# guangkun0818/speech2text

Measured on AMD Instinct MI355X. Metric: audio-seconds/sec (train step, zipformer pruned-RNN-T), higher is better.
Workload: dtype f32; 1 GPU; C3 zipformer pruned-RNN-T train step: chunk_size -1, 500 BPE, prune_range 5 (fbank+fwd+bwd+allreduce+ScaledAdam); accumulate_grad_batches=1, gemm_arith=bf16x2/3, per_gpu_batch=64, global_batch=64, labels_per_utt=50, parallelism=dp1

## Files before the change

include/s2t_mi355.h:

```cpp
#ifndef S2T_MI355_H_
#define S2T_MI355_H_

#ifdef __cplusplus
extern "C" {
#endif

int s2t_fbank_f32(const float* pcm, long pcm_stride, const long* num_samples, int batch,
                  const float* window400, const float* twiddle512, const int* mel_off,
                  const int* mel_k0, const float* mel_w, int nnz, int num_mel, float eps,
                  float scale_in, const float* cmvn_mean, const float* cmvn_istd, float* out,
                  int max_frames, long* out_frames, void* stream);

#define S2T_CTC_MAX_LABELS 1023
long s2t_ctc_workspace_floats(int B, int T, int Umax);
int s2t_ctc_loss_fwd_bwd(const float* logits, const long* targets, long tgt_stride,
                         const long* in_len, const long* tgt_len, int B, int T, int V, int Umax,
                         int blank, int zero_infinity, const float* grad_scale, float* workspace,
                         float* loss_per_utt, float* grad_logits, void* stream);

int s2t_fill_f32(float* p, long n, float v, void* stream);
int s2t_rnnt_row_exp(const float* x, long rows, int C, float* probs, float* rowmax, void* stream);
int s2t_rnnt_simple_pxpy(const float* am, const float* lm, const float* am_max,
                         const float* lm_max, const float* nrm, const long* symbols,
                         const long* boundary, int B, int S, int T, int C, int blank, float* px,
// ... 14 lines not shown
                         const float* lm_max, const float* nrm, const float* lm_sum,
                         const float* am_dot, const float* log_u, const long* symbols,
                         const long* boundary, int B, int S, int T, int C, int blank, float lam,
                         float mu, float* px, float* py, void* stream);
int s2t_rnnt_smooth_bwd(const float* am_probs, const float* lm_probs, const float* G_am,
                        const float* G_lm, const float* dpx, const float* dpy,
                        const float* gscale, const long* symbols, const float* lm_sum,
                        const float* am_dot, const float* u, int B, int S, int T, int C, int blank,
                        float lam, float mu, float* dlogu_part, float* v, float* d_am, float* d_lm,
                        void* stream);
int s2t_mutual_info_fwd(const float* px, const float* py, const long* boundary, int B, int S,
                        int T, float* p, float* ans, void* stream);
int s2t_mutual_info_bwd(const float* px, const float* py, const long* boundary, const float* p,
                        const float* ans_grad, int B, int S, int T, float* px_grad,
                        float* py_grad, void* stream);
int s2t_rnnt_prune_ranges(const float* px_grad, const float* py_grad, const long* boundary, int B,
                          int S, int T, int s_range, long* ranges, void* stream);
int s2t_rnnt_pruned_fwd(const float* am, const float* lm, const long* ranges,
                        const long* symbols, const long* boundary, int B, int S, int T, int C,
                        int R, int blank, int act, float* px, float* py, float* lse, void* stream);
int s2t_rnnt_pruned_bwd(const float* am, const float* lm, const long* ranges,
                        const long* symbols, const float* lse, const float* dpx, const float* dpy,
                        const float* gscale, int B, int S, int T, int C, int R, int blank, int act,
                        float* d_am, float* d_lm, int accumulate, void* stream);
int s2t_rnnt_lattice_fwd(const float* logits, const long* ranges, const long* symbols,
                         const long* boundary, int B, int S, int T, int V, int R, int blank,
                         float* px, float* py, float* lse, void* stream);
int s2t_rnnt_lattice_bwd(const float* logits, const long* ranges, const long* symbols,
                         const float* lse, const float* dpx, const float* dpy,
                         const float* gscale, int B, int S, int T, int V, int R, int blank,
                         float* d_logits, void* stream);


int s2t_swoosh_fwd(const float* x, float* y, long n, float offset, float constant, void* stream);
int s2t_swoosh_bwd(const float* x, const float* g, float* d, long n, float offset, void* stream);
int s2t_biasnorm_fwd(const float* x, const float* bias, const float* log_scale, long rows, int D,
                     float* y, float* scales, void* stream);
int s2t_biasnorm_fwd_tb(const float* x, const float* bias, const float* log_scale, int T, int B, int D,
                        float* y, float* scales, void* stream);
int s2t_biasnorm_bwd_tb(const float* x, const float* bias, const float* scales, const float* g, int T,
                        int B, int D, float* dx, float* dbias, float* dls, void* stream);
int s2t_norm_bypass_fwd(const float* x, const float* bias, const float* log_scale, const float* orig,
                        const float* bypass_scale, const float* fm, int B, long rows, int D, float* out,
                        float* scales, void* stream);
int s2t_norm_bypass_bwd(const float* x, const float* bias, const float* scales, const float* orig,
                        const float* bypass_scale, const float* g, const float* fm, int B, long rows, int D,
                        float* dx, float* d_orig, float* d_bypass_scale, float* dbias, float* dls,
                        void* stream);
int s2t_biasnorm_bwd(const float* x, const float* bias, const float* scales, const float* g,
                     long rows, int D, float* dx, float* dbias, float* dls, void* stream);
long s2t_balancer_bwd_workspace_floats(void);
int s2t_balancer_bwd(const float* x, long ldx, const float* g, long ldg, long rows, int C,
                     float min_mean, float max_mean, float min_rms, float max_rms,
                     float grad_scale, float* out, long ldo, float* workspace, int parity,
                     float act_off, void* stream);
int s2t_balancer_stats(const float* x, long ldx, long rows, int C, float* stats, void* stream);
int s2t_balancer_apply(const float* x, long ldx, const float* g, long ldg, long rows, int C,
                       float min_mean, float max_mean, float min_rms, float max_rms,
                       float grad_scale, float* out, long ldo, const float* stats, float act_off,
                       void* stream);


int s2t_zipconv_fwd(const float* u, long ld, int gate_off, const unsigned char* mask, int T, int B,
                    int C, int K, int chunk, const float* wc, const float* bc, const float* wk,
                    const float* bk, const float* scale, float* y, void* stream);
int s2t_zipconv_fwd_act(const float* u, long ld, int gate_off, const unsigned char* mask, int T, int B,
                        int C, int K, int chunk, const float* wc, const float* bc, const float* wk,
                        const float* bk, const float* scale, float* y, float* y_act, int act_kind,
                        void* stream);
int s2t_zipconv_bwd(const float* u, long ld, int gate_off, const unsigned char* mask, int T, int B,
                    int C, int K, int chunk, const float* wc, const float* wk, const float* bk,
                    const float* scale, const float* dy, float* du, float* dwc, float* dbc,
                    float* dwk, float* dbk, float* dscale, float* workspace, void* stream);
int s2t_zipconv_bwd_data(const float* u, long ld, int gate_off, const unsigned char* mask, int T,
                         int B, int C, int K, int chunk, const float* wc, const float* wk,
                         const float* bk, const float* scale, const float* dy, float* du,
                         void* stream);
int s2t_zipconv_bwd_params(const float* u, long ld, int gate_off, const unsigned char* mask, int T,
                           int B, int C, int K, int chunk, const float* wc, const float* wk,
                           const float* bk, const float* scale, const float* dy, float* dwc,
                           float* dbc, float* dwk, float* dbk, float* dscale, float* workspace,
                           void* stream);
long s2t_zipconv_bwd_workspace_floats(int T, int B, int C, int K);


int s2t_relpos_attn_fwd(const float* qkp, const float* pos, const unsigned char* kpm,
                        const unsigned char* amask, int T, int B, int H, int qd, int pd, float* W,
                        void* stream);
int s2t_relpos_attn_fwd_flag(const float* qkp, const float* pos, const unsigned char* kpm,
                             const unsigned char* amask, int T, int B, int H, int qd, int pd,
                             float* W, float pen_limit, float* pen_flag, void* stream);
int s2t_relpos_attn_bwd(const float* qkp, const float* pos, const unsigned char* kpm,
                        const unsigned char* amask, int T, int B, int H, int qd, int pd,
                        const float* W, const float* dW, const float* dW0, const float* dO1,
                        const float* V1, int dv1, const float* dO2, const float* V2, int dv2,
                        int delta_given, float* delta_ws, float* dqkp, float* dpos,
                        float* workspace, void* stream);
long s2t_relpos_attn_bwd_workspace_floats(int T, int B, int H, int pd);
int s2t_attn_apply(const float* W, const float* v, int T, int B, int H, int dv, int transpose,
                   float* out, void* stream);


long s2t_linear_wgrad_workspace_floats(int R, int N, int M);
int s2t_linear_wgrad(const float* g, long ldg, const float* a, long lda, int R, int N, int M,
                     float* dW, float* db, int accumulate, float* workspace, void* stream);

int s2t_whiten_metric(float* xtx, float* colsum, long n, int G, int cg, float* cov, float* mean,
                      float* scal, float* host_metric, float* workspace, void* stream);
int s2t_whiten_prep(const float* cov, const float* mean, const float* scal, int G, int cg, float* dcov,
                    float* bias, float* sums64, void* stream);
int s2t_gemm_x3p_sq(const float* A, long lda, const unsigned short* Bp, int N, int K, float* C, long ldc,
                    int M, const float* bias, const float* other, long ld_other, float* sums, int tile,
                    void* stream);
int s2t_sumsq64(const float* g, long numel, float* sums64, void* stream);
int s2t_whiten_combine64(const float* g, const float* pg, long numel, float grad_scale,
                         const float* sums64, float* out, void* stream);
int s2t_whiten_dcov(const float* cov, const float* mean, const float* scal, int G, int cg,
                    float* dcov, float* bias, float* sums, void* stream);
int s2t_whiten_apply(const float* g, const float* pg, long numel, float grad_scale, float* sums,
                     float* out, void* stream);
int s2t_limit_param_grad(const float* x, const float* g, float lo, float hi, long n, float* out,
                         void* stream);

int s2t_bestrq_labels(const float* feats, int B, int T, int F, const float* proj, int D,
                      const float* codebooks, int ncb, int K, int T2, long* labels, void* stream);


int s2t_col2im3x3_nhwc(const float* dc, int B, int H, int W, int C, int Ho, int Wo, int sh, int sw,
                       float* dx, void* stream);

int s2t_conv3x3_c1(int mode, const float* x, const float* w, const float* bias, const float* g, int B,
                   int H, int W, int pw, int CO, float* y, float* dw, float* db, float* dx,
                   void* stream);

int s2t_conv3x3_s2(int mode, const float* x, const float* w, const float* bias, const float* g, int B,
                   int H, int W, int CI, int CO, float* y, float* dx, void* stream);

int s2t_conv3x3_gemm(int mode, const float* x, int B, int H, int W, int C, int sh, int sw, int CO,
                     const float* w2_or_g, const float* bias, float* out, float* db, void* stream);

int s2t_dwconv2d_nhwc_fwd(const float* x, const float* wgt, const float* bias, int N, int H, int W,
                          int C, int KH, int KW, int flip, float* y, void* stream);
int s2t_dwconv2d_nhwc_fwd_add(const float* x, const float* wgt, const float* bias, const float* add,
                              int N, int H, int W, int C, int KH, int KW, int flip, float* y,
                              void* stream);
long s2t_dwconv2d_wgrad_workspace_floats(int N, int H, int C, int KH, int KW);
int s2t_dwconv2d_nhwc_wgrad(const float* x, const float* dy, int N, int H, int W, int C, int KH,
                            int KW, float* workspace, float* dw, float* db, void* stream);

int s2t_optim_chunk_elems(void);
int s2t_optim_segc_floats(void);
int s2t_seg_stats(const float* p, const float* g, const int* chunk_off, const int* chunk_len,
                  int nchunks, float* partial, void* stream);
int s2t_scaled_adam_coef(const float* partial, const int* seg_chunk_begin, const int* seg_len,
                         int nchunks_all, int seg_lo, int seg_hi, float lr, float beta1,
                         float beta2, float eps, float scalar_lr_scale, float param_min_rms,
                         float param_max_rms, float scalar_max, float clip_val,
                         float clipping_scale, int step, int size_update_period,
                         int clipping_update_period, float bc2, float bc2_size, float beta2c,
                         float* param_rms, float* scale_exp_avg_sq, float* scale_grads,
                         float* model_norms, float* fstate, int* istate, float* segstat,
                         float* segc, const float* skip, void* stream);
int s2t_scaled_adam_apply(float* p, float* g, float* delta, float* exp_avg_sq,
                          const int* chunk_off, const int* chunk_len, const int* chunk_seg,
                          int nchunks, const float* segc, int zero_grad, void* stream);

// ... 444 lines not shown
```

speech2text_amd/csrc/zip_conv.hip:

```cpp
#include "common.h"
#include <algorithm>
#include <cstdint>
#include <cstdlib>

namespace {

constexpr int TT = 64;
constexpr int FPT = 16;

__device__ __forceinline__ float sigmoidf_(float x) { return 1.f / (1.f + __expf(-x)); }

__device__ __forceinline__ float edge_scale(const float* __restrict__ s_le,
                                            const float* __restrict__ s_re, int c, int pos,
                                            int chunk, int K) {
  float sc = 1.f;
  if (pos < K) sc += s_le[pos * 64 + c];
  const int idx = pos - chunk + K;
  if (idx >= 0 && idx < K) sc += s_re[idx * 64 + c];
  return sc;
}

struct ConvArgs {
  const float* u;
  long ld;
// ... 389 lines not shown
#pragma unroll
      for (int i = 0; i < FPT; ++i) acc[i] = fmaf(w, win[i + 2 * halo - j], acc[i]);
    }
  } else if constexpr (SB > 0) {
#pragma unroll
    for (int sb = 0; sb < FPT / SB; ++sb) {
      constexpr int WM = SB + K - 1;
      const int i0 = sb * SB, lo = ((tb + i0) / chunk) * chunk - (tb - halo + i0);
      float wm[WM];
#pragma unroll
      for (int w = 0; w < WM; ++w) wm[w] = (w >= lo && w < lo + chunk) ? win[i0 + w] : 0.f;
#pragma unroll
      for (int j = 0; j < K; ++j) {
        const float w = s_wk[j * 64 + c];
#pragma unroll
        for (int i = 0; i < SB; ++i) acc[i0 + i] = fmaf(w, wm[i + 2 * halo - j], acc[i0 + i]);
      }
    }
  } else {
    int cs[FPT];
#pragma unroll
    for (int i = 0; i < FPT; ++i) cs[i] = ((tb + i) / chunk) * chunk;
#pragma unroll
    for (int j = 0; j < K; ++j) {
      const float w = s_wk[j * 64 + c];
#pragma unroll
      for (int i = 0; i < FPT; ++i) {
        const int t = tb + i + halo - j;
        if (t >= cs[i] && t < cs[i] + chunk) acc[i] = fmaf(w, win[i + 2 * halo - j], acc[i]);
      }
    }
  }
  if (vec) {
    __syncthreads();
#pragma unroll
    for (int i = 0; i < FPT; ++i) s_g[(tg * FPT + i) * 64 + c] = acc[i];
    __syncthreads();
#pragma unroll
    for (int p = 0; p < TT / 16; ++p) {
      const int r = 16 * p + rig, t = t0 + r;
      if (t >= a.T || ch >= a.C) continue;
      const float4 d = *reinterpret_cast<const float4*>(&s_g[r * 64 + 4 * c4]);
      const float dv[4] = {d.x, d.y, d.z, d.w};
      float* o = du + ((long)t * a.B + b) * nout + ch;
      const bool pad = qpad[p] != 0;
      if (gated) {
        const float xv[4] = {__uint_as_float(qx[p].x), __uint_as_float(qx[p].y), __uint_as_float(qx[p].z),
                             __uint_as_float(qx[p].w)};
        const float sv[4] = {__uint_as_float(qs[p].x), __uint_as_float(qs[p].y), __uint_as_float(qs[p].z),
                             __uint_as_float(qs[p].w)};
        float ox[4], og[4];
#pragma unroll
        for (int e = 0; e < 4; ++e) {
          const float sg = sigmoidf_(sv[e]);
          ox[e] = pad ? 0.f : dv[e] * sg;
          og[e] = pad ? 0.f : dv[e] * xv[e] * sg * (1.f - sg);
        }
        *reinterpret_cast<float4*>(o) = make_float4(ox[0], ox[1], ox[2], ox[3]);
        *reinterpret_cast<float4*>(o + a.C) = make_float4(og[0], og[1], og[2], og[3]);
      } else {
        *reinterpret_cast<float4*>(o) = pad ? make_float4(0.f, 0.f, 0.f, 0.f) : d;
      }
    }
    return;
  }
  if (!chan_ok) return;
#pragma unroll
  for (int i = 0; i < FPT; ++i) {
    const int t = tb + i;
    if (t < a.T) {
      const bool pad = opad[i] != 0;
      float* o = du + ((long)t * a.B + b) * nout;
      if (gated) {
        const float xv = oxv[i], sg = sigmoidf_(osv[i]);
        o[c0 + c] = pad ? 0.f : acc[i] * sg;
        o[a.C + c0 + c] = pad ? 0.f : acc[i] * xv * sg * (1.f - sg);
      } else {
        o[c0 + c] = pad ? 0.f : acc[i];
      }
    }
  }
}

template <int K, bool GEN, bool EDGE, int SB = 0>
__global__ __launch_bounds__(256) void zipconv_bwd_w_kernel(ConvArgs a,
                                                            const float* __restrict__ dy, int BB,
                                                            float* __restrict__ part,
                                                            float* __restrict__ dscale,
                                                            float* __restrict__ dscale_t = nullptr,
                                                            int cpad = 0) {
  constexpr int Kh = (K + 1) / 2, halo = K / 2, W = FPT + 2 * halo, NV = Kh + K + 2;
  extern __shared__ __attribute__((aligned(16))) unsigned char smem_raw[];
  float* s_x = reinterpret_cast<float*>(smem_raw);
  float* s_wc = s_x + (TT + 2 * halo) * 64;
  float* s_wk = s_wc + Kh * 64;
  float* s_le = EDGE ? s_wk + K * 64 : nullptr;
  float* s_re = EDGE ? s_le + K * 64 : nullptr;
  float* s_red = s_wk + (EDGE ? 3 : 1) * K * 64;
  const int tz = tile_z(a);
  const int c0 = blockIdx.x * 64, t0 = tz * TT;
  const int c = threadIdx.x & 63, tg = __builtin_amdgcn_readfirstlane(threadIdx.x >> 6);
  const int tb = t0 + tg * FPT;
  const int chunk = a.chunk;
  stage_weights<K>(a, c0, s_wc, s_wk, s_le, s_re,
                   EDGE && (GEN || t0 - K / 2 < K || t0 + TT + K / 2 > a.T - K));
  float pwc[Kh], pwk[K];
#pragma unroll
  for (int j = 0; j < Kh; ++j) pwc[j] = 0.f;
#pragma unroll
  for (int j = 0; j < K; ++j) pwk[j] = 0.f;
  float pbc = 0.f, pbk = 0.f;
  const bool chan_ok = c0 + c < a.C;
  int cs[FPT];
  float sc[FPT];
#pragma unroll
  for (int i = 0; i < FPT; ++i) {
    cs[i] = GEN ? ((tb + i) / chunk) * chunk : 0;
    sc[i] = 1.f;
  }
  __syncthreads();
  if (EDGE && a.scale) {
#pragma unroll
    for (int i = 0; i < FPT; ++i)
      if (tb + i < a.T) sc[i] = edge_scale(s_le, s_re, c, tb + i - cs[i], chunk, K);
  }
  bool edge = false;
  if (EDGE && dscale != nullptr) {
    const int p0 = t0 % chunk;
    edge = (p0 < K) || (p0 + TT - 1 >= chunk - K) || (p0 + TT > chunk);
  }
  const float bkv = (a.bk && chan_ok) ? a.bk[c0 + c] : 0.f;
  float ds[FPT];
#pragma unroll
  for (int i = 0; i < FPT; ++i) ds[i] = 0.f;
  const int b_end = min(a.B, (int)(blockIdx.y + 1) * BB);
  for (int b = blockIdx.y * BB; b < b_end; ++b) {
    __syncthreads();
    float gpre[FPT];
#pragma unroll
    for (int i = 0; i < FPT; ++i)
      gpre[i] = dy[((long)min(tb + i, a.T - 1) * a.B + b) * a.C + (chan_ok ? c0 + c : 0)];
    if (buf_ok(a)) stage_xg_buf<K>(a, b, t0, c0, s_x);
    else stage_xg<K>(a, b, t0, c0, s_x);
    __syncthreads();
    if (!chan_ok) continue;
    float win[W];
#pragma unroll
    for (int w = 0; w < W; ++w) win[w] = s_x[(tg * FPT + w) * 64 + c];
    if constexpr (GEN && SB > 0) {
#pragma unroll
      for (int i = 0; i < FPT; ++i) {
        const float g = (tb + i < a.T) ? gpre[i] : 0.f;
        pbc += g;
        pbk += g * sc[i];
        if (a.wc) {
#pragma unroll
          for (int j = 0; j < Kh; ++j) pwc[j] = fmaf(g, win[i + j], pwc[j]);
        }
      }
#pragma unroll
      for (int sb = 0; sb < FPT / SB; ++sb) {
        constexpr int WM = SB + K - 1;
        const int i0 = sb * SB, lo = cs[i0] - (tb - halo + i0);
        float wm[WM];
#pragma unroll
        for (int w = 0; w < WM; ++w) wm[w] = (w >= lo && w < lo + chunk) ? win[i0 + w] : 0.f;
        if (edge) {
          float ak[SB];
#pragma unroll
          for (int i = 0; i < SB; ++i) ak[i] = bkv;
#pragma unroll
          for (int j = 0; j < K; ++j) {
            const float w = s_wk[j * 64 + c];
#pragma unroll
            for (int i = 0; i < SB; ++i) ak[i] = fmaf(w, wm[i + j], ak[i]);
          }
#pragma unroll
          for (int i = 0; i < SB; ++i)
            if (tb + i0 + i < a.T) ds[i0 + i] = fmaf(gpre[i0 + i], ak[i], ds[i0 + i]);
        }
#pragma unroll
        for (int i = 0; i < SB; ++i) {
          const float gs = ((tb + i0 + i < a.T) ? gpre[i0 + i] : 0.f) * sc[i0 + i];
#pragma unroll
          for (int j = 0; j < K; ++j) pwk[j] = fmaf(gs, wm[i + j], pwk[j]);
        }
      }
    } else {
    if (edge) {
      float ak[FPT];
#pragma unroll
      for (int i = 0; i < FPT; ++i) ak[i] = bkv;
#pragma unroll
      for (int j = 0; j < K; ++j) {
        const float w = s_wk[j * 64 + c];
#pragma unroll
        for (int i = 0; i < FPT; ++i) {
          const int tt = tb + i - halo + j;
          if (!GEN || (tt >= cs[i] && tt < cs[i] + chunk)) ak[i] = fmaf(w, win[i + j], ak[i]);
        }
      }
#pragma unroll
      for (int i = 0; i < FPT; ++i)
        if (tb + i < a.T) ds[i] = fmaf(gpre[i], ak[i], ds[i]);
    }
#pragma unroll
    for (int i = 0; i < FPT; ++i) {
      const int t = tb + i;
      const float g = (t < a.T) ? gpre[i] : 0.f;
      const float gs = g * sc[i];
      pbc += g;
      pbk += gs;
      if (a.wc) {
#pragma unroll
        for (int j = 0; j < Kh; ++j) pwc[j] = fmaf(g, win[i + j], pwc[j]);
      }
#pragma unroll
      for (int j = 0; j < K; ++j) {
        if (!GEN) {
          pwk[j] = fmaf(gs, win[i + j], pwk[j]);
        } else {
          const int tt = t - halo + j;
          if (tt >= cs[i] && tt < cs[i] + chunk) pwk[j] = fmaf(gs, win[i + j], pwk[j]);
        }
      }
    }
    }
  }
  if (edge && chan_ok) {
#pragma unroll
    for (int i = 0; i < FPT; ++i) {
      const int t = tb + i;
      if (t >= a.T) continue;
      const int pos = t - cs[i], idx = pos - chunk + K;
      if (dscale_t) {
        if (pos < K) atomicAdd(&dscale_t[(long)pos * cpad + c0 + c], ds[i]);
        if (idx >= 0 && idx < K) atomicAdd(&dscale_t[((long)K + idx) * cpad + c0 + c], ds[i]);
      } else {
        if (pos < K) atomicAdd(&dscale[(long)(c0 + c) * K + pos], ds[i]);
        if (idx >= 0 && idx < K) atomicAdd(&dscale[((long)a.C + c0 + c) * K + idx], ds[i]);
      }
    }
  }
  const long blk = ((long)blockIdx.x * gridDim.y + blockIdx.y) * a.nt + tz;
  float* dst = part + blk * NV * 64 + c;
  auto reduce_store = [&](float v, int slot) {
    __syncthreads();
    s_red[tg * 64 + c] = v;
    __syncthreads();
    if (tg == 0) dst[slot * 64] = s_red[c] + s_red[64 + c] + s_red[128 + c] + s_red[192 + c];
  };
#pragma unroll
  for (int j = 0; j < Kh; ++j) reduce_store(pwc[j], j);
  reduce_store(pbc, Kh);
#pragma unroll
  for (int j = 0; j < K; ++j) reduce_store(pwk[j], Kh + 1 + j);
  reduce_store(pbk, Kh + 1 + K);
}

__global__ __launch_bounds__(256) void zipconv_reduce_w_kernel(
    const float* __restrict__ part, int nblk_per_ctile, int C, int Kh, int K,
    float* __restrict__ dwc, float* __restrict__ dbc, float* __restrict__ dwk,
    float* __restrict__ dbk) {
  __shared__ float s_red[4][64];
  const int NV = Kh + K + 2;
  const int ct = blockIdx.x, slot = blockIdx.y;
  const int c = threadIdx.x & 63, kg = threadIdx.x >> 6;
  float s = 0.f;
  const float* base = part + ((long)ct * nblk_per_ctile * NV + slot) * 64 + c;
  const long stride = (long)NV * 64;
  int k = kg;
  for (; k + 28 < nblk_per_ctile; k += 32) {
    float t[8];
#pragma unroll
    for (int u = 0; u < 8; ++u) t[u] = base[(k + 4 * u) * stride];
#pragma unroll
    for (int u = 0; u < 8; ++u) s += t[u];
  }
  for (; k < nblk_per_ctile; k += 4) s += base[k * stride];
  s_red[kg][c] = s;
  __syncthreads();
  const int cg = ct * 64 + c;
  if (kg == 0 && cg < C) {
    s = s_red[0][c] + s_red[1][c] + s_red[2][c] + s_red[3][c];
    if (slot < Kh) {
      if (dwc) dwc[(long)cg * Kh + slot] += s;
    } else if (slot == Kh) {
      if (dbc) dbc[cg] += s;
    } else if (slot < Kh + 1 + K) {
      dwk[(long)cg * K + slot - Kh - 1] += s;
    } else if (dbk) {
      dbk[cg] += s;
    }
  }
}

template <int K>
size_t conv_smem(bool with_red, int tiles, bool edge) {
  constexpr int Kh = (K + 1) / 2, halo = K / 2;
  return sizeof(float) * ((edge ? tiles : 1) * (TT + 2 * halo) * 64 + Kh * 64 + (edge ? 3 : 1) * K * 64 +
                          (with_red ? 256 : 0));
}

}

#define S2T_CONV_DISPATCH(K, BODY)  \
  switch (K) {                      \
    case 3: { constexpr int KK = 3; BODY; } break;   \
    case 5: { constexpr int KK = 5; BODY; } break;   \
    case 7: { constexpr int KK = 7; BODY; } break;   \
    case 15: { constexpr int KK = 15; BODY; } break; \
    case 31: { constexpr int KK = 31; BODY; } break; \
    default: return -1;             \
  }

static int conv_args_ok(int T, int B, int C, int K, int chunk) {
  return T > 0 && B > 0 && C > 0 && (K & 1) && chunk > 0;
}

struct ConvTiles {
  int nt;
  bool edge;
  ConvTiles(int T, bool gen, bool has_scale) : nt((T + TT - 1) / TT), edge(gen || has_scale) {}
};

static int conv_subblock(int chunk) {
  return (chunk >= 2 && (chunk & (chunk - 1)) == 0) ? std::min(chunk, FPT) : 0;
}
#define S2T_CONV_GEN_SB(SBSEL, LAUNCH) \
  switch (SBSEL) {                     \
    case 16: { constexpr int SBV = 16; LAUNCH; } break; \
    case 8: { constexpr int SBV = 8; LAUNCH; } break;   \
    case 4: { constexpr int SBV = 4; LAUNCH; } break;   \
    case 2: { constexpr int SBV = 2; LAUNCH; } break;   \
    default: { constexpr int SBV = 0; LAUNCH; } break;  \
  }

static int zipconv_fwd_impl(const float* u, long ld, int gate_off, const unsigned char* mask,
                            int T, int B, int C, int K, int chunk, const float* wc,
                            const float* bc, const float* wk, const float* bk,
                            const float* scale, float* y, float* y2, float act_off, float act_c,
                            void* stream) {
  if (!conv_args_ok(T, B, C, K, chunk)) return -1;
  ConvArgs a{u, ld, gate_off, mask, T, B, C, chunk, wc, bc, wk, bk, scale, 0, 1 << 30, 0, 0};
  hipStream_t st = (hipStream_t)stream;
  const bool gen = chunk < T;
  const ConvTiles z(T, gen, scale != nullptr);
  const unsigned gx = (C + 63) / 64;
  a.nt = z.nt;
  if (!z.edge) {
    S2T_CONV_DISPATCH(K, hipLaunchKernelGGL((zipconv_fwd_kernel<KK, false, false>), dim3(gx, B, z.nt),
                                            dim3(256), conv_smem<KK>(false, 1, false), st, a, y, y2, act_off, act_c));
    S2T_CHECK_LAUNCH();
  } else {
    const dim3 grid(gx, B, z.nt);
    if (!gen) {
      S2T_CONV_DISPATCH(K, hipLaunchKernelGGL((zipconv_fwd_kernel<KK, false, true>), grid, dim3(256),
                                              conv_smem<KK>(false, 1, true), st, a, y, y2, act_off, act_c));
    } else {
      S2T_CONV_GEN_SB(conv_subblock(chunk),
                      S2T_CONV_DISPATCH(K, hipLaunchKernelGGL((zipconv_fwd_kernel<KK, true, true, SBV>), grid,
                                                              dim3(256), conv_smem<KK>(false, 1, true), st, a, y,
                                                              y2, act_off, act_c)));
    }
    S2T_CHECK_LAUNCH();
  }
  return 0;
}

extern "C" int s2t_zipconv_fwd(const float* u, long ld, int gate_off, const unsigned char* mask,
                               int T, int B, int C, int K, int chunk, const float* wc,
                               const float* bc, const float* wk, const float* bk,
                               const float* scale, float* y, void* stream) {
  return zipconv_fwd_impl(u, ld, gate_off, mask, T, B, C, K, chunk, wc, bc, wk, bk, scale, y, nullptr, 0.f, 0.f,
                          stream);
}

extern "C" int s2t_zipconv_fwd_act(const float* u, long ld, int gate_off, const unsigned char* mask,
                                   int T, int B, int C, int K, int chunk, const float* wc,
                                   const float* bc, const float* wk, const float* bk,
                                   const float* scale, float* y, float* y_act, int act_kind,
                                   void* stream) {
  if (!y_act || (act_kind != 1 && act_kind != 2)) return -1;
  return zipconv_fwd_impl(u, ld, gate_off, mask, T, B, C, K, chunk, wc, bc, wk, bk, scale, y, y_act,
                          act_kind == 1 ? 4.0f : 1.0f, act_kind == 1 ? 0.035f : 0.313261687f, stream);
}

__global__ __launch_bounds__(256) void zipconv_dscale_commit_kernel(const float* __restrict__ t, int C,
                                                                    int K, int cpad,
                                                                    float* __restrict__ dscale) {
  const int i = blockIdx.x * 256 + threadIdx.x;
  if (i >= 2 * C * K) return;
  const int side = i / (C * K), c = (i / K) % C, p = i % K;
  const float v = t[((long)side * K + p) * cpad + c];
  if (v != 0.f) dscale[i] += v;
}

static long zipconv_part_floats(int T, int B, int C, int K) {
  const long tiles = (long)((T + TT - 1) / TT) * ((C + 63) / 64);
  return tiles * B * 64 * ((K + 1) / 2 + K + 2);
}
extern "C" long s2t_zipconv_bwd_workspace_floats(int T, int B, int C, int K) {
  return zipconv_part_floats(T, B, C, K) + 2L * K * ((C + 63) / 64) * 64;
}

static int zipconv_bwd_launch_data(ConvArgs a, int T, int B, int C, int K, bool gen, const ConvTiles& z,
                                   const float* dy, float* du, hipStream_t st) {
  const unsigned gx = (C + 63) / 64;
  a.nt = z.nt;
  if (!z.edge) {
    S2T_CONV_DISPATCH(K, hipLaunchKernelGGL((zipconv_bwd_data_kernel<KK, false, false>),
                                            dim3(gx, B, z.nt), dim3(256),
                                            conv_smem<KK>(false, 1, false), st, a, dy, du));
    S2T_CHECK_LAUNCH();
  } else {
    const dim3 grid(gx, B, z.nt);
    if (!gen) {
      S2T_CONV_DISPATCH(K, hipLaunchKernelGGL((zipconv_bwd_data_kernel<KK, false, true>), grid, dim3(256),
                                              conv_smem<KK>(false, 1, true), st, a, dy, du));
    } else {
      S2T_CONV_GEN_SB(conv_subblock(a.chunk),
                      S2T_CONV_DISPATCH(K, hipLaunchKernelGGL((zipconv_bwd_data_kernel<KK, true, true, SBV>), grid,
                                                              dim3(256), conv_smem<KK>(false, 1, true), st, a, dy,
                                                              du)));
    }
    S2T_CHECK_LAUNCH();
  }
  return 0;
}

static int zipconv_bwd_launch_params(ConvArgs a, int T, int B, int C, int K, bool gen, const ConvTiles& z,
                                     const float* wc, const float* scale, const float* dy, float* dwc,
                                     float* dbc, float* dwk, float* dbk, float* dscale,
                                     float* workspace, hipStream_t st) {
  const unsigned gx = (C + 63) / 64;
  const long tiles = (long)gx * z.nt;
  const char* env = getenv("S2T_CONV_BLOCKS");
  int BB = (int)((tiles * B) / (env ? std::max(1, atoi(env)) : (K >= 31 ? 192 : 128)));
  if (BB < 1) BB = 1;
  if (BB > 16) BB = 16;
  const unsigned gy = (B + BB - 1) / BB;
  float* const dsc = (scale && dscale) ? dscale : nullptr;
  a.nt = z.nt;
  if (!z.edge) {
    S2T_CONV_DISPATCH(K, hipLaunchKernelGGL((zipconv_bwd_w_kernel<KK, false, false>), dim3(gx, gy, z.nt),
                                            dim3(256), conv_smem<KK>(true, 1, false), st, a, dy, BB,
                                            workspace, dsc));
    S2T_CHECK_LAUNCH();
  } else {
    const dim3 gridw(gx, gy, z.nt);
    if (!gen) {
      S2T_CONV_DISPATCH(K, hipLaunchKernelGGL((zipconv_bwd_w_kernel<KK, false, true>), gridw, dim3(256),
                                              conv_smem<KK>(true, 1, true), st, a, dy, BB, workspace, dsc));
    } else {
      const int cpad = (int)gx * 64;
      float* dst = dsc ? workspace + zipconv_part_floats(T, B, C, K) : nullptr;
      if (dst && hipMemsetAsync(dst, 0, sizeof(float) * 2 * K * cpad, st) != hipSuccess) return -3;
      S2T_CONV_GEN_SB(conv_subblock(a.chunk),
                      S2T_CONV_DISPATCH(K, hipLaunchKernelGGL((zipconv_bwd_w_kernel<KK, true, true, SBV>), gridw,
                                                              dim3(256), conv_smem<KK>(true, 1, true), st, a, dy, BB,
                                                              workspace, dsc, dst, cpad)));
      S2T_CHECK_LAUNCH();
      if (dst) hipLaunchKernelGGL(zipconv_dscale_commit_kernel, dim3((2 * C * K + 255) / 256), dim3(256), 0, st,
                                  dst, C, K, cpad, dsc);
    }
    S2T_CHECK_LAUNCH();
  }
  hipLaunchKernelGGL(zipconv_reduce_w_kernel, dim3(gx, (K + 1) / 2 + K + 2), dim3(256), 0,
                     st, workspace, (int)(z.nt * gy), C, (K + 1) / 2, K, wc ? dwc : nullptr,
                     wc ? dbc : nullptr, dwk, dbk);
  S2T_CHECK_LAUNCH();
  return 0;
}

extern "C" int s2t_zipconv_bwd(const float* u, long ld, int gate_off, const unsigned char* mask,
                               int T, int B, int C, int K, int chunk, const float* wc,
                               const float* wk, const float* bk, const float* scale,
                               const float* dy, float* du, float* dwc, float* dbc, float* dwk,
                               float* dbk, float* dscale, float* workspace, void* stream) {
  if (!conv_args_ok(T, B, C, K, chunk)) return -1;
  hipStream_t st = (hipStream_t)stream;
  ConvArgs a{u, ld, gate_off, mask, T, B, C, chunk, wc, nullptr, wk, bk, scale, 0, 1 << 30, 0, 0};
  const bool gen = chunk < T;
  const ConvTiles z(T, gen, scale != nullptr);
  const unsigned gx = (C + 63) / 64;
  int rc = zipconv_bwd_launch_data(a, T, B, C, K, gen, z, dy, du, st);
  if (rc != 0) return rc;
  return zipconv_bwd_launch_params(a, T, B, C, K, gen, z, wc, scale, dy, dwc, dbc, dwk, dbk, dscale,
                                   workspace, st);
}

extern "C" int s2t_zipconv_bwd_data(const float* u, long ld, int gate_off, const unsigned char* mask,
                                    int T, int B, int C, int K, int chunk, const float* wc,
                                    const float* wk, const float* bk, const float* scale,
                                    const float* dy, float* du, void* stream) {
  if (!conv_args_ok(T, B, C, K, chunk)) return -1;
  ConvArgs a{u, ld, gate_off, mask, T, B, C, chunk, wc, nullptr, wk, bk, scale, 0, 1 << 30, 0, 0};
  const bool gen = chunk < T;
  const ConvTiles z(T, gen, scale != nullptr);
  return zipconv_bwd_launch_data(a, T, B, C, K, gen, z, dy, du, (hipStream_t)stream);
}

extern "C" int s2t_zipconv_bwd_params(const float* u, long ld, int gate_off,
                                      const unsigned char* mask, int T, int B, int C, int K,
                                      int chunk, const float* wc, const float* wk, const float* bk,
                                      const float* scale, const float* dy, float* dwc, float* dbc,
                                      float* dwk, float* dbk, float* dscale, float* workspace,
                                      void* stream) {
  if (!conv_args_ok(T, B, C, K, chunk)) return -1;
  ConvArgs a{u, ld, gate_off, mask, T, B, C, chunk, wc, nullptr, wk, bk, scale, 0, 1 << 30, 0, 0};
  const bool gen = chunk < T;
  const ConvTiles z(T, gen, scale != nullptr);
  return zipconv_bwd_launch_params(a, T, B, C, K, gen, z, wc, scale, dy, dwc, dbc, dwk, dbk, dscale,
                                   workspace, (hipStream_t)stream);
}
```

Baseline: 18240 audio-seconds/sec.

## Add streaming per-run weight-gradient kernel for full-context zipformer conv backward

For the non-chunked case (chunk_size -1), the parameter-gradient pass now uses a new kernel. Each wave streams one long time run per utterance with a sliding register window and buffer loads, instead of tiled blocks that stage halos in shared memory. Separate blocks handle only the left and right edge positions, which need the scale and dscale terms, and a new reduction kernel combines the partial sums. The chunked kernel loses its GEN/EDGE template specialisations, so that path now always runs the chunk-masking and edge code. Risks include a larger workspace, 2GB buffer-offset limits, and extra branches in the chunked kernel.

```diff
diff --git a/include/s2t_mi355.h b/include/s2t_mi355.h
--- a/include/s2t_mi355.h
+++ b/include/s2t_mi355.h
@@ -120,6 +120,7 @@
                            float* dbc, float* dwk, float* dbk, float* dscale, float* workspace,
                            void* stream);
 long s2t_zipconv_bwd_workspace_floats(int T, int B, int C, int K);
+int s2t_zipconv_bwd_params_run(int K);
 
 
 int s2t_relpos_attn_fwd(const float* qkp, const float* pos, const unsigned char* kpm,
diff --git a/speech2text_amd/csrc/zip_conv.hip b/speech2text_amd/csrc/zip_conv.hip
--- a/speech2text_amd/csrc/zip_conv.hip
+++ b/speech2text_amd/csrc/zip_conv.hip
@@ -495,7 +495,7 @@
   }
 }
 
-template <int K, bool GEN, bool EDGE, int SB = 0>
+template <int K, int SB = 0>
 __global__ __launch_bounds__(256) void zipconv_bwd_w_kernel(ConvArgs a,
                                                             const float* __restrict__ dy, int BB,
                                                             float* __restrict__ part,
@@ -507,16 +507,15 @@
   float* s_x = reinterpret_cast<float*>(smem_raw);
   float* s_wc = s_x + (TT + 2 * halo) * 64;
   float* s_wk = s_wc + Kh * 64;
-  float* s_le = EDGE ? s_wk + K * 64 : nullptr;
-  float* s_re = EDGE ? s_le + K * 64 : nullptr;
-  float* s_red = s_wk + (EDGE ? 3 : 1) * K * 64;
+  float* s_le = s_wk + K * 64;
+  float* s_re = s_le + K * 64;
+  float* s_red = s_wk + 3 * K * 64;
   const int tz = tile_z(a);
   const int c0 = blockIdx.x * 64, t0 = tz * TT;
   const int c = threadIdx.x & 63, tg = __builtin_amdgcn_readfirstlane(threadIdx.x >> 6);
   const int tb = t0 + tg * FPT;
   const int chunk = a.chunk;
-  stage_weights<K>(a, c0, s_wc, s_wk, s_le, s_re,
-                   EDGE && (GEN || t0 - K / 2 < K || t0 + TT + K / 2 > a.T - K));
+  stage_weights<K>(a, c0, s_wc, s_wk, s_le, s_re, true);
   float pwc[Kh], pwk[K];
 #pragma unroll
   for (int j = 0; j < Kh; ++j) pwc[j] = 0.f;
@@ -528,17 +527,17 @@
   float sc[FPT];
 #pragma unroll
   for (int i = 0; i < FPT; ++i) {
-    cs[i] = GEN ? ((tb + i) / chunk) * chunk : 0;
+    cs[i] = ((tb + i) / chunk) * chunk;
     sc[i] = 1.f;
   }
   __syncthreads();
-  if (EDGE && a.scale) {
+  if (a.scale) {
 #pragma unroll
     for (int i = 0; i < FPT; ++i)
       if (tb + i < a.T) sc[i] = edge_scale(s_le, s_re, c, tb + i - cs[i], chunk, K);
   }
   bool edge = false;
-  if (EDGE && dscale != nullptr) {
+  if (dscale != nullptr) {
     const int p0 = t0 % chunk;
     edge = (p0 < K) || (p0 + TT - 1 >= chunk - K) || (p0 + TT > chunk);
   }
@@ -560,7 +559,7 @@
     float win[W];
 #pragma unroll
     for (int w = 0; w < W; ++w) win[w] = s_x[(tg * FPT + w) * 64 + c];
-    if constexpr (GEN && SB > 0) {
+    if constexpr (SB > 0) {
 #pragma unroll
       for (int i = 0; i < FPT; ++i) {
         const float g = (tb + i < a.T) ? gpre[i] : 0.f;
@@ -610,7 +609,7 @@
 #pragma unroll
         for (int i = 0; i < FPT; ++i) {
           const int tt = tb + i - halo + j;
-          if (!GEN || (tt >= cs[i] && tt < cs[i] + chunk)) ak[i] = fmaf(w, win[i + j], ak[i]);
+          if (tt >= cs[i] && tt < cs[i] + chunk) ak[i] = fmaf(w, win[i + j], ak[i]);
         }
       }
 #pragma unroll
@@ -630,12 +629,8 @@
       }
 #pragma unroll
       for (int j = 0; j < K; ++j) {
-        if (!GEN) {
-          pwk[j] = fmaf(gs, win[i + j], pwk[j]);
-        } else {
-          const int tt = t - halo + j;
-          if (tt >= cs[i] && tt < cs[i] + chunk) pwk[j] = fmaf(gs, win[i + j], pwk[j]);
-        }
+        const int tt = t - halo + j;
+        if (tt >= cs[i] && tt < cs[i] + chunk) pwk[j] = fmaf(gs, win[i + j], pwk[j]);
       }
     }
     }
@@ -705,6 +700,315 @@
     } else if (dbk) {
       dbk[cg] += s;
     }
+  }
+}
+
+constexpr int PW = 4;
+constexpr int PQ = 6;
+constexpr int PQE = 3;
+constexpr int param_run(int K) { return K >= 31 ? 96 : 64; }
+constexpr int param_edge_groups(int K) { return K >= 31 ? 4 : 1; }
+
+struct ParamPlan {
+  int runs, len;
+  int nwi;
+  int nbg;
+};
+
+struct RowLd { float x, g; unsigned char m; };
+
+struct ParamSrc {
+  __amdgpu_buffer_rsrc_t u, m, d;
+  int us, gs, ds;
+  bool gated;
+};
+struct ParamCur { int x, g, d, m; };
+
+__device__ __forceinline__ int param_records(long bytes) { return (int)(bytes < 0x7FFFFFF0L ? bytes : 0x7FFFFFF0L); }
+__device__ __forceinline__ ParamSrc param_src(const ConvArgs& a, const float* dy, int b, int tlo) {
+  ParamSrc s;
+  const long rows = (long)(a.T - 1 - tlo) * a.B + 1;
+  s.u = __builtin_amdgcn_make_buffer_rsrc(const_cast<float*>(a.u + ((long)tlo * a.B + b) * a.ld), 0,
+                                          param_records(rows * a.ld * 4), 0x00020000);
+  s.d = __builtin_amdgcn_make_buffer_rsrc(const_cast<float*>(dy + ((long)tlo * a.B + b) * a.C), 0,
+                                          param_records(rows * a.C * 4), 0x00020000);
+  s.m = __builtin_amdgcn_make_buffer_rsrc(const_cast<unsigned char*>(a.mask ? a.mask + (long)b * a.T + tlo : a.mask),
+                                          0, a.mask ? a.T - tlo : 0, 0x00020000);
+  s.gated = a.gate_off >= 0;
+  s.us = a.B * (int)a.ld * 4;
+  s.gs = s.gated ? s.us : 0;
+  s.ds = a.B * a.C * 4;
+  return s;
+}
+__device__ __forceinline__ ParamCur param_cursor(const ConvArgs& a, const ParamSrc& s, int rx, int rd, int cc) {
+  ParamCur q;
+  q.x = rx * s.us + cc * 4;
+  q.g = s.gated ? rx * s.us + (a.gate_off + cc) * 4 : 0x7FFFFFF0;
+  q.d = rd * s.ds + cc * 4;
+  q.m = rx;
+  asm volatile("" : "+v"(q.x), "+v"(q.g), "+v"(q.d), "+v"(q.m));
+  return q;
+}
+__device__ __forceinline__ RowLd param_row_load(const ParamSrc& s, ParamCur& q) {
+  RowLd v;
+  v.x = __uint_as_float(__builtin_amdgcn_raw_buffer_load_b32(s.u, q.x, 0, 0));
+  v.g = __uint_as_float(__builtin_amdgcn_raw_buffer_load_b32(s.u, q.g, 0, 0));
+  v.m = __builtin_amdgcn_raw_buffer_load_b8(s.m, q.m, 0, 0);
+  q.x += s.us;
+  q.g += s.gs;
+  q.m += 1;
+  return v;
+}
+__device__ __forceinline__ float param_dy_load(const ParamSrc& s, ParamCur& q) {
+  const float g = __uint_as_float(__builtin_amdgcn_raw_buffer_load_b32(s.d, q.d, 0, 0));
+  q.d += s.ds;
+  return g;
+}
+__device__ __forceinline__ float param_row_value(const ParamSrc& s, const RowLd& v) {
+  const float x = v.x * (s.gated ? sigmoidf_(v.g) : 1.f);
+  return v.m ? 0.f : x;
+}
+
+template <int K>
+__device__ __forceinline__ void param_window_fill(const ParamSrc& s, ParamCur& q, float (&win)[K]) {
+  constexpr int NB = 6;
+  win[0] = 0.f;
+#pragma unroll
+  for (int j0 = 0; j0 < K - 1; j0 += NB) {
+    RowLd r[NB];
+#pragma unroll
+    for (int i = 0; i < NB; ++i)
+      if (j0 + i < K - 1) r[i] = param_row_load(s, q);
+#pragma unroll
+    for (int i = 0; i < NB; ++i)
+      if (j0 + i < K - 1) win[1 + j0 + i] = param_row_value(s, r[i]);
+    __builtin_amdgcn_sched_barrier(0);
+  }
+}
+
+template <int NS>
+__device__ __forceinline__ void param_fold_waves(float (&acc)[NS], float* s_buf, int wave, int c) {
+#pragma unroll
+  for (int s0 = 0; s0 < NS; s0 += 16) {
+    __syncthreads();
+    if (wave > 0) {
+#pragma unroll
+      for (int i = 0; i < 16; ++i)
+        if (s0 + i < NS) s_buf[((wave - 1) * 16 + i) * 64 + c] = acc[s0 + i];
+    }
+    __syncthreads();
+    if (wave == 0) {
+#pragma unroll
+      for (int i = 0; i < 16; ++i)
+        if (s0 + i < NS) {
+#pragma unroll
+          for (int w = 0; w < PW - 1; ++w) acc[s0 + i] += s_buf[(w * 16 + i) * 64 + c];
+        }
+    }
+  }
+}
+
+template <int K>
+__global__ __launch_bounds__(64 * PW, 4) void zipconv_bwd_p_kernel(ConvArgs a, const float* __restrict__ dy,
+                                                                 ParamPlan pl, int want_ds,
+                                                                 float* __restrict__ part) {
+  constexpr int halo = K / 2;
+  constexpr int HE = (K + param_edge_groups(K) - 1) / param_edge_groups(K);
+  constexpr int NSM = std::max(std::max(2 * K, (PW - 1) * 16), PW * HE) * 64;
+  static_assert(NSM * 4 <= 16384, "zipconv_bwd_p_kernel: LDS budget");
+  __shared__ float smem[NSM];
+  const int gx = (a.C + 63) / 64;
+  const int c = threadIdx.x & 63, wave = __builtin_amdgcn_readfirstlane(threadIdx.x >> 6);
+  const int nE = 2 * gx * pl.nbg;
+  const int blk = blockIdx.x;
+  if (blk >= nE) {
+    const int bi = blk - nE;
+    const int ct = bi % gx, w = bi / gx;
+    const int cc = min(ct * 64 + c, a.C - 1);
+    float acc[K + 1];
+#pragma unroll
+    for (int j = 0; j <= K; ++j) acc[j] = 0.f;
+    const int items = a.B * pl.runs;
+    for (int q = w * PW + wave; q < items; q += pl.nwi * PW) {
+      const int b = q % a.B, ta = (q / a.B) * pl.len;
+      const int n = min(a.T, ta + pl.len) - ta;
+      if (n <= 0) continue;
+      const int tlo = max(ta - halo, 0);
+      const ParamSrc src = param_src(a, dy, b, tlo);
+      ParamCur cur = param_cursor(a, src, ta - halo - tlo, ta - tlo, cc);
+      float win[K];
+      param_window_fill<K>(src, cur, win);
+      RowLd qr[PQ];
+      float qd[PQ];
+#pragma unroll
+      for (int i = 0; i < PQ; ++i) {
+        qr[i] = param_row_load(src, cur);
+        qd[i] = param_dy_load(src, cur);
+      }
+      for (int f0 = 0; f0 < n; f0 += K) {
+#pragma unroll
+        for (int p = 0; p < K; ++p) {
+          const int f = f0 + p;
+          if (f >= n) break;
+          const float v = param_row_value(src, qr[0]), g = qd[0];
+#pragma unroll
+          for (int i = 0; i < PQ - 1; ++i) {
+            qr[i] = qr[i + 1];
+            qd[i] = qd[i + 1];
+          }
+          qr[PQ - 1] = param_row_load(src, cur);
+          qd[PQ - 1] = param_dy_load(src, cur);
+#pragma unroll
+          for (int j = 0; j < K - 1; ++j) win[j] = win[j + 1];
+          win[K - 1] = v;
+#pragma unroll
+          for (int j = 0; j < K; ++j) acc[j] = fmaf(g, win[j], acc[j]);
+          acc[K] += g;
+          __builtin_amdgcn_sched_barrier(0);
+        }
+      }
+    }
+    param_fold_waves<K + 1>(acc, smem, wave, c);
+    if (wave == 0) {
+      float* dst = part + ((long)ct * pl.nwi + w) * (K + 1) * 64 + c;
+#pragma unroll
+      for (int j = 0; j <= K; ++j) dst[j * 64] = acc[j];
+    }
+    return;
+  }
+  const int ct = blk % gx, side = (blk / gx) & 1, bg = blk / (2 * gx);
+  const int c0 = ct * 64, cc = min(c0 + c, a.C - 1);
+  float* s_wk = smem;
+  float* s_sc = smem + K * 64;
+  for (int i = threadIdx.x; i < 64 * K; i += 64 * PW) {
+    const int ch = i / K, j = i % K, cg = min(c0 + ch, a.C - 1);
+    s_wk[j * 64 + ch] = a.wk[(long)cg * K + j];
+    s_sc[j * 64 + ch] = a.scale[((long)side * a.C + cg) * K + j];
+  }
+  __syncthreads();
+  constexpr int NG = param_edge_groups(K), WPG = PW / NG, H = (K + NG - 1) / NG;
+  const int grp = wave / WPG, lane_b = wave % WPG, p0 = grp * H;
+  const int tb0 = (side == 0 ? 0 : a.chunk - K) + p0;
+  const float bkv = a.bk ? a.bk[cc] : 0.f;
+  float acc[K + 1], ds[H];
+#pragma unroll
+  for (int j = 0; j <= K; ++j) acc[j] = 0.f;
+#pragma unroll
+  for (int j = 0; j < H; ++j) ds[j] = 0.f;
+  if (tb0 < a.T) {
+    for (int b = bg + pl.nbg * lane_b; b < a.B; b += pl.nbg * WPG) {
+      const int tlo = max(tb0 - halo, 0);
+      const ParamSrc src = param_src(a, dy, b, tlo);
+      ParamCur cur = param_cursor(a, src, tb0 - halo - tlo, tb0 - tlo, cc);
+      int lc = c;
+      asm volatile("" : "+v"(lc));
+      float win[K];
+      param_window_fill<K>(src, cur, win);
+      RowLd qr[PQE];
+      float qd[PQE];
+#pragma unroll
+      for (int i = 0; i < PQE; ++i) {
+        qr[i] = param_row_load(src, cur);
+        qd[i] = param_dy_load(src, cur);
+      }
+#pragma unroll
+      for (int i = 0; i < H; ++i) {
+        const int p = p0 + i;
+        if (p >= K) break;
+        const float v = param_row_value(src, qr[0]), g = qd[0];
+#pragma unroll
+        for (int q = 0; q < PQE - 1; ++q) {
+          qr[q] = qr[q + 1];
+          qd[q] = qd[q + 1];
+        }
+        if (i + PQE < H) {
+          qr[PQE - 1] = param_row_load(src, cur);
+          qd[PQE - 1] = param_dy_load(src, cur);
+        }
+#pragma unroll
+        for (int j = 0; j < K - 1; ++j) win[j] = win[j + 1];
+        win[K - 1] = v;
+        const float gs = g * s_sc[p * 64 + lc];
+#pragma unroll
+        for (int j = 0; j < K; ++j) asm("v_fmac_f32_e32 %0, %1, %2" : "+v"(acc[j]) : "v"(gs), "v"(win[j]));
+        acc[K] += gs;
+        if (want_ds) {
+          float ak = bkv;
+#pragma unroll
+          for (int j = 0; j < K; ++j) {
+            ak = fmaf(s_wk[j * 64 + lc], win[j], ak);
+            if ((j & 7) == 7) __builtin_amdgcn_sched_barrier(0);
+          }
+          ds[i] = fmaf(g, ak, ds[i]);
+        }
+        __builtin_amdgcn_sched_barrier(0);
+      }
+    }
+  }
+  param_fold_waves<K + 1>(acc, smem, wave, c);
+  __syncthreads();
+#pragma unroll
+  for (int i = 0; i < H; ++i) smem[(wave * H + i) * 64 + c] = ds[i];
+  __syncthreads();
+  float* dst = part + (long)gx * pl.nwi * (K + 1) * 64 +
+               (((long)side * gx + ct) * pl.nbg + bg) * (2 * K + 1) * 64 + c;
+  if (wave == 0) {
+#pragma unroll
+    for (int j = 0; j <= K; ++j) dst[j * 64] = acc[j];
+  }
+  if (lane_b == 0) {
+#pragma unroll
+    for (int i = 0; i < H; ++i) {
+      float v = smem[(wave * H + i) * 64 + c];
+#pragma unroll
+      for (int w = 1; w < WPG; ++w) v += smem[((wave + w) * H + i) * 64 + c];
+      if (p0 + i < K) dst[(K + 1 + p0 + i) * 64] = v;
+    }
+  }
+}
+
+__global__ __launch_bounds__(256) void zipconv_reduce_p_kernel(
+    const float* __restrict__ part, ParamPlan pl, int C, int K, float* __restrict__ dwc,
+    float* __restrict__ dbc, float* __restrict__ dwk, float* __restrict__ dbk,
+    float* __restrict__ dscale) {
+  __shared__ float s_red[2][4][64];
+  const int gx = (C + 63) / 64, Kh = (K + 1) / 2;
+  const int ct = blockIdx.x, slot = blockIdx.y;
+  const int c = threadIdx.x & 63, kg = threadIdx.x >> 6;
+  const float* pe = part + (long)gx * pl.nwi * (K + 1) * 64;
+  const long es = (long)(2 * K + 1) * 64;
+  float si = 0.f, se = 0.f;
+  if (slot <= K) {
+    const float* pi = part + ((long)ct * pl.nwi * (K + 1) + slot) * 64 + c;
+#pragma unroll 4
+    for (int k = kg; k < pl.nwi; k += 4) si += pi[(long)k * (K + 1) * 64];
+#pragma unroll 4
+    for (int k = kg; k < 2 * pl.nbg; k += 4) {
+      const int side = k / pl.nbg, bg = k % pl.nbg;
+      se += pe[(((long)side * gx + ct) * pl.nbg + bg) * es + slot * 64 + c];
+    }
+  } else {
+    const int side = (slot - K - 1) / K, p = (slot - K - 1) % K;
+#pragma unroll 4
+    for (int bg = kg; bg < pl.nbg; bg += 4)
+      se += pe[(((long)side * gx + ct) * pl.nbg + bg) * es + (K + 1 + p) * 64 + c];
+  }
+  s_red[0][kg][c] = si;
+  s_red[1][kg][c] = se;
+  __syncthreads();
+  const int cg = ct * 64 + c;
+  if (kg != 0 || cg >= C) return;
+  si = s_red[0][0][c] + s_red[0][1][c] + s_red[0][2][c] + s_red[0][3][c];
+  se = s_red[1][0][c] + s_red[1][1][c] + s_red[1][2][c] + s_red[1][3][c];
+  if (slot < K) {
+    dwk[(long)cg * K + slot] += si + se;
+    if (dwc && slot < Kh) dwc[(long)cg * Kh + slot] += si;
+  } else if (slot == K) {
+    if (dbk) dbk[cg] += si + se;
+    if (dbc) dbc[cg] += si;
+  } else {
+    const int side = (slot - K - 1) / K, p = (slot - K - 1) % K;
+    dscale[((long)side * C + cg) * K + p] += se;
   }
 }
 
@@ -809,14 +1113,6 @@
   if (v != 0.f) dscale[i] += v;
 }
 
-static long zipconv_part_floats(int T, int B, int C, int K) {
-  const long tiles = (long)((T + TT - 1) / TT) * ((C + 63) / 64);
-  return tiles * B * 64 * ((K + 1) / 2 + K + 2);
-}
-extern "C" long s2t_zipconv_bwd_workspace_floats(int T, int B, int C, int K) {
-  return zipconv_part_floats(T, B, C, K) + 2L * K * ((C + 63) / 64) * 64;
-}
-
 static int zipconv_bwd_launch_data(ConvArgs a, int T, int B, int C, int K, bool gen, const ConvTiles& z,
                                    const float* dy, float* du, hipStream_t st) {
   const unsigned gx = (C + 63) / 64;
@@ -842,43 +1138,99 @@
   return 0;
 }
 
+static ParamPlan param_plan_for(int T, int B, int C, int K, bool edge, long G) {
+  const long gx = (C + 63) / 64;
+  const int L = param_run(K);
+  ParamPlan pl;
+  pl.runs = (T + L - 1) / L;
+  pl.len = (T + pl.runs - 1) / pl.runs;
+  const long items = (long)B * pl.runs;
+  const long GE = edge ? std::max<long>(2 * gx, G * 5 * K / (T + 5 * K)) : 0;
+  const long GI = std::max<long>(gx, G - GE);
+  long nwi = GI / gx;
+  if (nwi * PW < items) {
+    const long m = (items + PW * nwi - 1) / (PW * nwi);
+    nwi = (items + PW * m - 1) / (PW * m);
+  }
+  long nbg = 0;
+  if (edge) {
+    const long wpg = PW / param_edge_groups(K);
+    nbg = GE / (2 * gx);
+    if (nbg * wpg < B) {
+      const long m = (B + wpg * nbg - 1) / (wpg * nbg);
+      nbg = (B + wpg * m - 1) / (wpg * m);
+    }
+  }
+  pl.nwi = (int)nwi;
+  pl.nbg = (int)nbg;
+  return pl;
+}
+static long param_plan_floats(const ParamPlan& pl, int C, int K) {
+  const long gx = (C + 63) / 64;
+  return gx * pl.nwi * (K + 1) * 64 + 2 * gx * pl.nbg * (2 * K + 1) * 64;
+}
+static long param_plan_wgs(const ParamPlan& pl, int C) { return (long)((C + 63) / 64) * (pl.nwi + 2 * pl.nbg); }
+
+constexpr long kParamBlocks = 512;
+
+static ParamPlan param_plan(int T, int B, int C, int K, bool edge, long cap, bool use_env) {
+  const char* env = use_env ? getenv("S2T_CONV_BLOCKS") : nullptr;
+  long G = env ? std::max(1, atoi(env)) : kParamBlocks;
+  if (!env) cap = std::min(cap, 3L * T * B * C / 20);
+  for (;;) {
+    const ParamPlan pl = param_plan_for(T, B, C, K, edge, G);
+    if ((param_plan_floats(pl, C, K) <= cap && param_plan_wgs(pl, C) <= std::max<long>(G, 1)) || G <= 1) return pl;
+    G = G * 7 / 8;
+  }
+}
+
+extern "C" int s2t_zipconv_bwd_params_run(int K) { return param_run(K); }
+
+static long zipconv_part_floats(int T, int B, int C, int K) {
+  const long tiles = (long)((T + TT - 1) / TT) * ((C + 63) / 64);
+  return tiles * B * 64 * ((K + 1) / 2 + K + 2);
+}
+extern "C" long s2t_zipconv_bwd_workspace_floats(int T, int B, int C, int K) {
+  const long chunked = zipconv_part_floats(T, B, C, K) + 2L * K * ((C + 63) / 64) * 64;
+  return std::max(chunked, param_plan_floats(param_plan_for(T, B, C, K, true, 1), C, K));
+}
+
 static int zipconv_bwd_launch_params(ConvArgs a, int T, int B, int C, int K, bool gen, const ConvTiles& z,
                                      const float* wc, const float* scale, const float* dy, float* dwc,
                                      float* dbc, float* dwk, float* dbk, float* dscale,
                                      float* workspace, hipStream_t st) {
   const unsigned gx = (C + 63) / 64;
+  float* const dsc = (scale && dscale) ? dscale : nullptr;
+  a.nt = z.nt;
+  if (!gen) {
+    if ((long)(param_run(K) + 2 * K + PQ) * B * std::max<long>(a.ld, C) * 4 >= 0x7FFFFFF0L) return -1;
+    const ParamPlan pl = param_plan(T, B, C, K, scale != nullptr, s2t_zipconv_bwd_workspace_floats(T, B, C, K), true);
+    S2T_CONV_DISPATCH(K, hipLaunchKernelGGL((zipconv_bwd_p_kernel<KK>), dim3((unsigned)param_plan_wgs(pl, C)),
+                                            dim3(64 * PW), 0, st, a, dy, pl, dsc ? 1 : 0, workspace));
+    S2T_CHECK_LAUNCH();
+    hipLaunchKernelGGL(zipconv_reduce_p_kernel, dim3(gx, K + 1 + (dsc ? 2 * K : 0)), dim3(256), 0, st, workspace,
+                       pl, C, K, wc ? dwc : nullptr, wc ? dbc : nullptr, dwk, dbk, dsc);
+    S2T_CHECK_LAUNCH();
+    return 0;
+  }
   const long tiles = (long)gx * z.nt;
   const char* env = getenv("S2T_CONV_BLOCKS");
   int BB = (int)((tiles * B) / (env ? std::max(1, atoi(env)) : (K >= 31 ? 192 : 128)));
   if (BB < 1) BB = 1;
   if (BB > 16) BB = 16;
   const unsigned gy = (B + BB - 1) / BB;
-  float* const dsc = (scale && dscale) ? dscale : nullptr;
-  a.nt = z.nt;
-  if (!z.edge) {
-    S2T_CONV_DISPATCH(K, hipLaunchKernelGGL((zipconv_bwd_w_kernel<KK, false, false>), dim3(gx, gy, z.nt),
-                                            dim3(256), conv_smem<KK>(true, 1, false), st, a, dy, BB,
-                                            workspace, dsc));
-    S2T_CHECK_LAUNCH();
-  } else {
-    const dim3 gridw(gx, gy, z.nt);
-    if (!gen) {
-      S2T_CONV_DISPATCH(K, hipLaunchKernelGGL((zipconv_bwd_w_kernel<KK, false, true>), gridw, dim3(256),
-                                              conv_smem<KK>(true, 1, true), st, a, dy, BB, workspace, dsc));
-    } else {
-      const int cpad = (int)gx * 64;
-      float* dst = dsc ? workspace + zipconv_part_floats(T, B, C, K) : nullptr;
-      if (dst && hipMemsetAsync(dst, 0, sizeof(float) * 2 * K * cpad, st) != hipSuccess) return -3;
-      S2T_CONV_GEN_SB(conv_subblock(a.chunk),
-                      S2T_CONV_DISPATCH(K, hipLaunchKernelGGL((zipconv_bwd_w_kernel<KK, true, true, SBV>), gridw,
-                                                              dim3(256), conv_smem<KK>(true, 1, true), st, a, dy, BB,
-                                                              workspace, dsc, dst, cpad)));
-      S2T_CHECK_LAUNCH();
-      if (dst) hipLaunchKernelGGL(zipconv_dscale_commit_kernel, dim3((2 * C * K + 255) / 256), dim3(256), 0, st,
-                                  dst, C, K, cpad, dsc);
-    }
-    S2T_CHECK_LAUNCH();
-  }
+  const dim3 gridw(gx, gy, z.nt);
+  const int cpad = (int)gx * 64;
+  float* dst = dsc ? workspace + zipconv_part_floats(T, B, C, K) : nullptr;
+  if (dst && hipMemsetAsync(dst, 0, sizeof(float) * 2 * K * cpad, st) != hipSuccess) return -3;
+  S2T_CONV_GEN_SB(conv_subblock(a.chunk),
+                  S2T_CONV_DISPATCH(K, hipLaunchKernelGGL((zipconv_bwd_w_kernel<KK, SBV>), gridw,
+                                                          dim3(256), conv_smem<KK>(true, 1, true), st, a, dy, BB,
+                                                          workspace, dsc, dst, cpad)));
+  S2T_CHECK_LAUNCH();
+  if (dst) hipLaunchKernelGGL(zipconv_dscale_commit_kernel, dim3((2 * C * K + 255) / 256), dim3(256), 0, st,
+                              dst, C, K, cpad, dsc);
+  S2T_CHECK_LAUNCH();
   hipLaunchKernelGGL(zipconv_reduce_w_kernel, dim3(gx, (K + 1) / 2 + K + 2), dim3(256), 0,
                      st, workspace, (int)(z.nt * gy), C, (K + 1) / 2, K, wc ? dwc : nullptr,
                      wc ? dbc : nullptr, dwk, dbk);
```

Measured after the change: 18380 audio-seconds/sec, median of 6. About the same (+0.7%).
